# hynkis/Python-MPC

Measured on AMD Instinct MI355X. Metric: QP solves/sec (batch) at N=20 nx=4 nu=1, higher is better.
Workload: dtype f64

## Files before the change

### python-mpc_amd/csrc/device_common.h

```cpp
#pragma once
#include <hip/hip_runtime.h>

#include "kernels.h"

#ifdef MPCQP_SKEW
__device__ inline __attribute__((convergent)) void mpcqp_skew_barrier() {
    __builtin_amdgcn_fence(__ATOMIC_RELEASE, "workgroup");
    __builtin_amdgcn_s_barrier();
    __builtin_amdgcn_fence(__ATOMIC_ACQUIRE, "workgroup");
    const unsigned w = __builtin_amdgcn_readfirstlane(threadIdx.x >> 6);
    const unsigned t = (unsigned)(__builtin_amdgcn_s_memtime() >> 3);
    if (((t ^ (w * 0x9E3779B9u)) >> 7) & 1u) __builtin_amdgcn_s_sleep(20);
}
#define __syncthreads() mpcqp_skew_barrier()
#endif

namespace mpcqp {

#define OSQP_INFTY 1e30
#define MIN_SCALING 1e-4
#define MAX_SCALING 1e4
#define RHO_MIN 1e-6
#define RHO_MAX 1e6
#define RHO_TOL 1e-4
// ... 26 lines not shown
template <int CTRL>
__device__ __forceinline__ double dpp(double v) {
    int lo = __double2loint(v), hi = __double2hiint(v);
    lo = __builtin_amdgcn_mov_dpp(lo, CTRL, 0xF, 0xF, true);
    hi = __builtin_amdgcn_mov_dpp(hi, CTRL, 0xF, 0xF, true);
    return __hiloint2double(hi, lo);
}

__device__ __forceinline__ double reduce8(double v) {
    v += dpp<0xB1>(v);
    v += dpp<0x4E>(v);
    v += dpp<0x141>(v);
    return v;
}

__device__ __forceinline__ double reduce16(double v) {
    v += dpp<0xB1>(v);
    v += dpp<0x4E>(v);
    v += dpp<0x141>(v);
    v += dpp<0x140>(v);
    return v;
}

template <int CTRL, int RM>
__device__ __forceinline__ double dpp_rows(double v) {
    int lo = __double2loint(v), hi = __double2hiint(v);
    lo = __builtin_amdgcn_mov_dpp(lo, CTRL, RM, 0xF, true);
    hi = __builtin_amdgcn_mov_dpp(hi, CTRL, RM, 0xF, true);
    return __hiloint2double(hi, lo);
}

__device__ __forceinline__ double reduce32_hi(double v) {
    v = reduce16(v);
    v += dpp_rows<0x142, 0xA>(v);
    return v;
}

__device__ __forceinline__ double lane63(double v) {
    return __hiloint2double(__builtin_amdgcn_readlane(__double2hiint(v), 63),
                            __builtin_amdgcn_readlane(__double2loint(v), 63));
}
__device__ __forceinline__ double wave_max(double v) {
    v = cmax(v, dpp<0xB1>(v));
    v = cmax(v, dpp<0x4E>(v));
    v = cmax(v, dpp<0x141>(v));
    v = cmax(v, dpp<0x140>(v));
    v = cmax(v, dpp_rows<0x142, 0xA>(v));
    v = cmax(v, dpp_rows<0x143, 0xC>(v));
    return lane63(v);
}
__device__ __forceinline__ double wave_sum(double v) {
    v = reduce16(v);
    v += dpp_rows<0x142, 0xA>(v);
    v += dpp_rows<0x143, 0xC>(v);
    return lane63(v);
}

template <int TT, int K>
__device__ __forceinline__ void block_max(double (&v)[K], double* red) {
    if constexpr (TT == 64) {
#pragma unroll
        for (int k = 0; k < K; ++k) v[k] = wave_max(v[k]);
    } else {
        constexpr int NW = TT / 64;
        const int wid = threadIdx.x >> 6, lane = threadIdx.x & 63;
#pragma unroll
        for (int k = 0; k < K; ++k) {
            const double r = wave_max(v[k]);
            if (lane == 0) red[wid * K + k] = r;
        }
        __syncthreads();
#pragma unroll
        for (int k = 0; k < K; ++k) {
            double r = red[k];
#pragma unroll
            for (int w = 1; w < NW; ++w) r = cmax(r, red[w * K + k]);
            v[k] = r;
        }
        __syncthreads();
    }
}

template <int TT, int K>
__device__ __forceinline__ void block_max_to(const double (&v)[K], double* red, double* out) {
    constexpr int NW = TT / 64;
    const int wid = threadIdx.x >> 6, lane = threadIdx.x & 63, t = threadIdx.x;
#pragma unroll
    for (int k = 0; k < K; ++k) {
        const double r = wave_max(v[k]);
        if (lane == 0) red[wid * K + k] = r;
    }
    __syncthreads();
    if (t < K) {
        double r = red[t];
#pragma unroll
        for (int w = 1; w < NW; ++w) r = cmax(r, red[w * K + t]);
        out[t] = r;
    }
    __syncthreads();
}

template <int TT, int K>
__device__ __forceinline__ void block_sum(double (&v)[K], double* red) {
    if constexpr (TT == 64) {
#pragma unroll
        for (int k = 0; k < K; ++k) v[k] = wave_sum(v[k]);
    } else {
        constexpr int NW = TT / 64;
        const int wid = threadIdx.x >> 6, lane = threadIdx.x & 63;
#pragma unroll
        for (int k = 0; k < K; ++k) {
            const double r = wave_sum(v[k]);
            if (lane == 0) red[wid * K + k] = r;
        }
        __syncthreads();
#pragma unroll
        for (int k = 0; k < K; ++k) {
            double r = red[k];
            if constexpr (NW == 4) {
                r = (red[k] + red[K + k]) + (red[2 * K + k] + red[3 * K + k]);
            } else {
#pragma unroll
                for (int w = 1; w < NW; ++w) r += red[w * K + k];
            }
            v[k] = r;
        }
        __syncthreads();
    }
}

__device__ __forceinline__ double vmax(double a, double b) { return __builtin_fmax(a, b); }

template <int CTRL, int K>
__device__ __forceinline__ void tmax_step(const double (&in)[K], double (&out)[(K + 1) / 2], bool upper) {
    constexpr int H = (K + 1) / 2;
#pragma unroll
    for (int j = 0; j < H; ++j) {
        const double lo = in[j];
        const double hi = j + H < K ? in[j + H] : 0.0;
        out[j] = vmax(upper ? hi : lo, dpp<CTRL>(upper ? lo : hi));
    }
}

template <bool HALF>
__device__ __forceinline__ double xmax_swap(double v) {
    const unsigned lo = (unsigned)__double2loint(v), hi = (unsigned)__double2hiint(v);
    const auto l = HALF ? __builtin_amdgcn_permlane32_swap(lo, lo, false, false)
                        : __builtin_amdgcn_permlane16_swap(lo, lo, false, false);
    const auto h = HALF ? __builtin_amdgcn_permlane32_swap(hi, hi, false, false)
                        : __builtin_amdgcn_permlane16_swap(hi, hi, false, false);
    return vmax(__hiloint2double((int)h[0], (int)l[0]), __hiloint2double((int)h[1], (int)l[1]));
}

template <int TT, int K, int KS>
__device__ __forceinline__ void block_max_sum_tr(double (&v)[K], double (&sm)[KS], double* red) {
    constexpr int NW = TT / 64, K1 = (K + 1) / 2, K2 = (K1 + 1) / 2;
    const int lane = threadIdx.x & 63, wid = threadIdx.x >> 6;
    double t1[K1], t2[K2];
    tmax_step<0xB1, K>(v, t1, lane & 1);
    tmax_step<0x4E, K1>(t1, t2, (lane >> 1) & 1);
#pragma unroll
    for (int j = 0; j < K2; ++j) {
        double x = t2[j];
        x = vmax(x, dpp<0x124>(x));
        x = vmax(x, dpp<0x128>(x));
        x = xmax_swap<false>(x);
        x = xmax_swap<true>(x);
        t2[j] = x;
    }
    double s[KS];
#pragma unroll
    for (int k = 0; k < KS; ++k) s[k] = wave_sum(sm[k]);
    double* rs = red + 4 * NW * K2;
    if (lane < 4) {
        int lq = lane;
        asm volatile("" : "+v"(lq));
#pragma unroll
        for (int j = 0; j < K2; ++j) red[(lq * K2 + j) * NW + wid] = t2[j];
    }
    if (lane == 0) {
        int wq = wid;
        asm volatile("" : "+v"(wq));
#pragma unroll
        for (int k = 0; k < KS; ++k) rs[wq * KS + k] = s[k];
    }
    __syncthreads();
    if constexpr (NW > 4) {
        double* const fin = rs + NW * KS;
        if ((int)threadIdx.x < K) {
            const int k = threadIdx.x, b0 = k >= K1, r1 = k - K1 * b0, b1 = r1 >= K2, j = r1 - K2 * b1;
            const double* src = red + ((b0 + 2 * b1) * K2 + j) * NW;
            double r = src[0];
#pragma unroll
            for (int w = 1; w < NW; ++w) r = vmax(r, src[w]);
            fin[k] = r;
        }
        __syncthreads();
#pragma unroll
        for (int k = 0; k < K; ++k) v[k] = fin[k];
    } else {
#pragma unroll
        for (int k = 0; k < K; ++k) {
            const int b0 = k >= K1, r1 = k - K1 * b0, b1 = r1 >= K2, j = r1 - K2 * b1;
            const double* src = red + ((b0 + 2 * b1) * K2 + j) * NW;
            double r = src[0];
#pragma unroll
            for (int w = 1; w < NW; ++w) r = vmax(r, src[w]);
            v[k] = r;
        }
    }
#pragma unroll
    for (int k = 0; k < KS; ++k) {
        double r = rs[k];
        if constexpr (NW == 4) {
            r = (rs[k] + rs[KS + k]) + (rs[2 * KS + k] + rs[3 * KS + k]);
        } else {
#pragma unroll
            for (int w = 1; w < NW; ++w) r += rs[w * KS + k];
        }
        sm[k] = r;
    }
    __syncthreads();
}

template <int TT>
__device__ __forceinline__ void order_epilogue(const KParams& p, int* smem) {
    const long B = gridDim.x;
    if (!p.done || !p.order || B <= p.slots || B > kOrderFuseMax) return;
    const int tid = threadIdx.x;
    int* cnt = smem;
    int* last = smem + 256;
    __syncthreads();
    if (tid == 0) {
        __threadfence();
        *last = atomicAdd(p.done, 1) == (int)(B - 1);
        __threadfence();
    }
    __syncthreads();
    if (!*last) return;
    int shift = 0;
    while ((p.max_iter >> shift) >= 256) ++shift;
    const int* iter = p.iter;
    int* order = const_cast<int*>(p.order);
    auto bin = [&](long i) {
        const int k = __builtin_nontemporal_load(iter + i) >> shift;
        return 255 - (k < 255 ? k : 255);
    };
    for (int k = tid; k < 256; k += TT) cnt[k] = 0;
    __syncthreads();
    for (long i = tid; i < B; i += TT) atomicAdd(&cnt[bin(i)], 1);
    __syncthreads();
    if (tid == 0) {
        int s = 0;
        for (int k = 0; k < 256; ++k) {
            const int c = cnt[k];
            cnt[k] = s;
            s += c;
        }
        *p.done = 0;
    }
    __syncthreads();
    for (long i = tid; i < B; i += TT) order[atomicAdd(&cnt[bin(i)], 1)] = (int)i;
}

template <int TT>
__device__ __forceinline__ bool block_any(bool f, int* flag) {
    if constexpr (TT == 64) {
        return __builtin_amdgcn_ballot_w64(f) != 0;
    } else {
        if (threadIdx.x == 0) *flag = 0;
        __syncthreads();
        if (f) *flag = 1;
        __syncthreads();
        bool r = *flag != 0;
        __syncthreads();
        return r;
    }
}

}
```

### python-mpc_amd/csrc/solve_wave.hip

```cpp
#include <hip/hip_runtime.h>

#include <algorithm>
#include <cstdlib>
#include <type_traits>

#include "setup_r.h"
#include "solve_phases.h"
#include "wave_util.h"

namespace mpcqp {

[[maybe_unused]] constexpr int TW = 64;

#ifdef MPCQP_EXPERIMENTAL
struct WaveFactor {
    double SB[2][S];
    __device__ __forceinline__ void load(const double* __restrict__ Sg) {
        const int lane = threadIdx.x, h = lane >> 5, r = lane & 31;
#pragma unroll
        for (int e = 0; e < 2; ++e) {
            const double* src = Sg + (long)(e ? 3 - h : h) * SS + r * S;
#pragma unroll
            for (int c = 0; c < S; ++c) SB[e][c] = src[c];
        }
// ... 855 lines not shown
#endif
            p.prof[b * kProfSlots + 6] = clock64() - t0c;
            p.prof[b * kProfSlots + 7] = wall_clock64() - t0w;
            p.prof[b * kProfSlots + 15] = t0w;
        }
    }
#endif
#undef PH
#undef PHL
#undef PHC
}

template <int K, int RS, int KPK, int K1>
__global__ __launch_bounds__(T2, 1) void k_solve_w2(KParams p, double* __restrict__ xo, double* __restrict__ yo,
                                                    int factor_only) {
    solve_w2_body<K, RS, KPK, K1>(p, xo, yo, factor_only);
    extern __shared__ __attribute__((aligned(16))) double sm[];
    order_epilogue<T2>(p, (int*)sm);
}

template <int K, int RS, int KPK, int K1, int SK, int SRS, int SAS, int SPS>
__global__ __launch_bounds__(T2, 1) void k_setup_solve_w2(KParams p, const double* __restrict__ Px_in,
                                                          const double* __restrict__ Ax_in,
                                                          const double* __restrict__ q_in,
                                                          const double* __restrict__ l_in,
                                                          const double* __restrict__ u_in, double* __restrict__ xo,
                                                          double* __restrict__ yo) {
    extern __shared__ __attribute__((aligned(16))) double sm[];
    setup_r_body<T2, SK, 4, SRS, SAS, SPS>(p, instance_of(p), Px_in, Ax_in, q_in, l_in, u_in, sm);
    __syncthreads();
    solve_w2_body<K, RS, KPK, K1>(p, xo, yo, 0);
    order_epilogue<T2>(p, (int*)sm);
}

constexpr int T4 = 256;

template <int QR, int NB0, int NB1>
__device__ __forceinline__ void form_dense_rows(__attribute__((address_space(1))) dpair* kd, const double* Sg,
                                                const double* gl, int a, int lane) {
    constexpr int NP = 6, T4_ = 256, TC = 8;
    auto pidx = [](int x, int y) { return y < x ? x * (x - 1) / 2 + y : NP; };
    const int bq = lane >> 4, l16 = lane & 15, i0 = 4 * (l16 >> 1);
    const double* const Ta = Sg + a * SS;
    const int nbs = (bq >> 1) ? NB1 : NB0, jb = (bq >> 1) ? NB0 : 0;
    const unsigned t0 = (unsigned)(a * 64 + (bq & 1) * 32 + i0);
#pragma unroll 1
    for (int pass = 0; pass < 2; ++pass) {
        const int c0 = 16 * (l16 & 1) + TC * pass;
        double acc[4][TC];
        {
            const double* src = Sg + bq * SS + i0 * S + c0;
            const bool diag = bq == a;
#pragma unroll
            for (int i = 0; i < 4; ++i)
#pragma unroll
                for (int c = 0; c < TC; c += 2) {
                    double v0, v1;
                    ld2(src + i * S + c, v0, v1);
                    acc[i][c] = diag ? v0 : 0.0;
                    acc[i][c + 1] = diag ? v1 : 0.0;
                }
        }
        auto step = [&](const double (&cf)[4], const double* row) __attribute__((always_inline)) {
            double rv[TC];
#pragma unroll
            for (int c = 0; c < TC; c += 2) ld2(row + c, rv[c], rv[c + 1]);
#pragma unroll
            for (int i = 0; i < 4; ++i)
#pragma unroll
                for (int c = 0; c < TC; ++c) acc[i][c] += cf[i] * rv[c];
        };
        if (a > 0) {
            const double* g = gl + pidx(a, bq) * 8 * S + c0;
#pragma unroll
            for (int q = 0; q < QR; ++q) {
                double cf[4];
#pragma unroll
                for (int i = 0; i < 4; ++i) cf[i] = Ta[(i0 + i) * S + q];
                step(cf, g + q * S);
            }
        }
        if (a < 3) {
            const double* g = gl + pidx(bq, a) * 8 * S + i0;
            const double* Tb = Sg + bq * SS + c0;
#pragma unroll
            for (int q = 0; q < QR; ++q) {
                double cf[4];
                ld2(g + q * S, cf[0], cf[1]);
                ld2(g + q * S + 2, cf[2], cf[3]);
                step(cf, Tb + q * S);
            }
        }
#pragma unroll 1
        for (int k = a + 1; k < 4; ++k) {
            const double* gka = gl + pidx(k, a) * 8 * S + i0;
            const double* gkb = gl + pidx(k, bq) * 8 * S + c0;
            const double* Tk = Sg + k * SS;
            double V[4][QR];
#pragma unroll
            for (int i = 0; i < 4; ++i)
#pragma unroll
                for (int q = 0; q < QR; ++q) V[i][q] = 0.0;
#pragma unroll
            for (int pp = 0; pp < QR; ++pp) {
                double g[4];
                ld2(gka + pp * S, g[0], g[1]);
                ld2(gka + pp * S + 2, g[2], g[3]);
#pragma unroll
                for (int q = 0; q < QR; ++q) {
                    const double t = Tk[pp * S + q];
#pragma unroll
                    for (int i = 0; i < 4; ++i) V[i][q] += g[i] * t;
                }
            }
#pragma unroll
            for (int q = 0; q < QR; ++q) {
                const double cf[4] = {V[0][q], V[1][q], V[2][q], V[3][q]};
                step(cf, gkb + q * S);
            }
        }
#pragma unroll
        for (int c = 0; c < TC; c += 2) {
            if (c0 + c < nbs) {
                const unsigned jp = (unsigned)((jb + c0 + c) >> 1);
#pragma unroll
                for (int i = 0; i < 4; ++i) {
                    kd[jp * T4_ + t0 + i].x = acc[i][c];
                    kd[jp * T4_ + t0 + i].y = acc[i][c + 1];
                }
            }
        }
    }
}

template <int K, int KPK, int QR, bool EL = false, int KC = K, bool DK = false, bool RU = false, bool ONE = false,
          int GL = 0>
__device__ __forceinline__ void solve_w4_body(const KParams& p, double* __restrict__ xo, double* __restrict__ yo,
                                              int factor_only = 0) {
    static_assert(!(DK && EL), "the dense inverse covers plans without eliminated columns");
    const int tid = threadIdx.x, w = __builtin_amdgcn_readfirstlane(tid >> 6), lane = tid & 63;
    const int h = lane >> 5, r = lane & 31;
    constexpr int NB = 4, NP = NB * (NB - 1) / 2;
    static_assert(KC % 2 == 0, "the rhs splits the column list over the half-waves");
    constexpr int KH = KC / 2;
    constexpr int LE = 2;
    const long b = instance_of(p);
    const int n = p.n, m = p.m, npad = p.npad, nnzP = p.nnzP, nnzA = p.nnzA;
    SL2 C = carve(p);
    SLds& L = C.L;
    const double* Hg = GL == 1 ? C.L.Acsc + 2 * ((lds_base_bytes(p) + 15) / 16) + (long)NB * SS
                           : p.H + b * (long)p.nb * SS;
    double* const Sg = C.L.Acsc + 2 * ((lds_base_bytes(p) + 15) / 16);
    constexpr bool SWZ = ONE && GL == 1 && !EL && !DK && QR <= 5;

    if (p.err[b]) {
        for (int j = tid; j < n; j += T4) if (xo) xo[b * n + j] = __builtin_nan("");
        for (int i = tid; i < m; i += T4) if (yo) yo[b * m + i] = __builtin_nan("");
        if (tid == 0) fail_status(p, b);
        return;
    }
#ifdef MPCQP_PHASE_PROF
    long long tph = 0, t0c = 0, t0w = 0;
    const bool prof = p.prof != nullptr;
    if (prof) { t0w = wall_clock64(); t0c = tph = clock64(); if (tid < 16) L.pacc[tid] = 0; }
#define PH(k) if (prof && tid == 0) { const long long t_ = clock64(); L.pacc[k] += t_ - tph; tph = t_; }
#else
#define PH(k)
#endif
    constexpr bool OPQ = EL || QR > 5;
    auto cscal = [&](int k) __attribute__((always_inline)) {
        return OPQ ? opaque_gptr(p.scal + b * 4)[k] : p.scal[b * 4 + k];
    };
    double rho = p.scal[b * 4 + 2];
    const double sigma = p.sigma, alpha = p.alpha;
    const bool warm = !ONE && p.warm_start != 0;
    const int mp = solve_mpad(m);
    if constexpr (!ONE) {
        for (int e = tid; e < nnzA; e += T4) L.Acsc[e] = p.Ax[b * nnzA + e];
        if (tid == 0) L.Acsc[nnzA] = 0.0;
        for (int v = tid; v < nnzP; v += T4) L.Pv[v] = p.Px[b * nnzP + v];
        if (tid == 0) L.Pv[nnzP] = 0.0;
        for (int i = tid; i < mp; i += T4) {
            const bool in = i < m;
            L.lo[i] = in ? p.l[b * m + i] : 0.0;
            L.up[i] = in ? p.u[b * m + i] : 0.0;
            L.ct[i] = in ? p.ct[b * m + i] : 0;
            C.Z[i] = (in && warm) ? p.z[b * m + i] : 0.0;
        }
        for (int pc = tid; pc < npad; pc += T4) {
            L.qv[pc] = p.q[b * npad + pc];
            C.X[pc] = warm ? p.x[b * npad + pc] : 0.0;
        }
    } else {
        if (tid == 0) L.Acsc[nnzA] = 0.0;
        if (tid == 0) L.Pv[nnzP] = 0.0;
        if constexpr (GL == 2)
            for (int o = tid; o < (NP + 1) * 8 * S; o += T4) L.gl[o] = 0.0;
    }
    if (tid < 8) L.cor[tid] = 0.0;
    if (tid < 8) L.cor[32 + tid] = 0.0;
    if (tid < 16) L.res[tid] = 0.0;
    if (tid < 4) L.flag[tid] = 0;

    int status = MPCQP_UNSOLVED_, rho_updates = 0, iter = 0, info_iter = 0;
    bool can_check = false, need_factor = true;
    const bool low = h == 0;
    const int pe0 = (EL && !low) ? p.eown[w * S + r] : -1;
    const bool colv = low && p.pad_var[w * S + r] >= 0;
    double* const Fo = p.F + b * (long)p.nb * SS;
    double ec = 0.0, ed = 0.0;
    const unsigned abase = lds_addr(L.Acsc), wbase = lds_addr(L.w), xbase = lds_addr(L.xt);
    const unsigned Xbase = lds_addr(C.X);
    GatherW<K> rg;
    GatherW<KH> chs;
    GatherW<LE> el;
    const bool rows_wave = w * 64 < mp;
    constexpr int NB0 = 26, NB1 = 28;
    static_assert(!DK || (NB0 + NB1) * T4 == kDenseRowDoubles, "KParams::Kd rows");
    double Kr[DK ? NB0 + NB1 : 1];
    constexpr int DKW = 8;
    PH(5)
    for (;;) {
        const int tid = OPQ ? opaque_v(threadIdx.x) : (int)threadIdx.x;
        const int lane = tid & 63, h = lane >> 5, r = lane & 31, rr = lane >> 3, ch = lane & 7;
        const int pc = w * S + r;
        const int pe = OPQ ? opaque_v(pe0) : pe0;
        const int xc = pe >= 0 ? pe : pc;
        const int ri = min(tid, mp - 1);
        __syncthreads();
        if (need_factor) {
            need_factor = false;
            if (iter > 0) {
                if constexpr (GL == 1) {
                    double* const ysv = Sg + (long)NB * SS + (long)(NB * (NB - 1) / 2) * p.amax * S;
                    for (int i = tid; i < m; i += T4) ysv[i] = L.ys[i];
                } else {
                    const auto yp = opaque_gptr(p.y + b * m);
                    for (int i = tid; i < m; i += T4) yp[i] = L.ys[i];
                }
                __syncthreads();
            }
            bool ok;
            if constexpr (RU) {
                if (iter == 0 && p.reuse && p.ffresh[b] == 1 && p.scal[b * 4 + 3] == rho) {
                    const double2* src = (const double2*)(p.Si + b * (long)p.nb * SS);
                    for (int e = tid; e < 2 * SS; e += T4) ((double2*)Sg)[e] = src[e];
                    ok = true;
                } else if constexpr (EL) {
                    ok = factorize_lds_nl<T4, EL>(p.self, b, rho);
                } else {
                    ok = factorize_nl<T4, EL>(p.self, b, rho, Sg);
                }
                __syncthreads();
                if (tid == 0) p.ffresh[b] = 0;
            } else if constexpr (GL == 1) {
                ok = factorize_g_nl<T4, EL, SWZ>(p.self, b, rho);
            } else if constexpr (GL == 2) {
                ok = factorize_gl_nl<T4, EL>(p.self, b, rho);
            } else if constexpr (EL) {
                ok = factorize_lds_nl<T4, EL>(p.self, b, rho);
            } else {
                ok = factorize_nl<T4, EL>(p.self, b, rho, Sg);
            }
            if (!ok) {
                if (iter == 0) {
                    if (xo) for (int j = tid; j < n; j += T4) opaque_ptr(xo + b * n)[j] = __builtin_nan("");
                    if (yo) for (int i = tid; i < m; i += T4) opaque_ptr(yo + b * m)[i] = __builtin_nan("");
                    if (tid == 0) fail_status(p, b);
                    return;
                }
                status = MPCQP_NON_CVX_;
                can_check = true;
                break;
            }
            if (factor_only) {
                __syncthreads();
                double2* dst = (double2*)(p.Si + b * (long)p.nb * SS);
                for (int e = tid; e < 2 * SS; e += T4) dst[e] = ((const double2*)Sg)[e];
                if (tid == 0) {
                    p.ffresh[b] = 1;
                    p.scal[b * 4 + 3] = rho;
                }
                return;
            }
            __syncthreads();
            const bool have_y = iter > 0 || warm;
            if constexpr (GL == 1) {
                const double* const ysv = Sg + (long)NB * SS + (long)(NB * (NB - 1) / 2) * p.amax * S;
                for (int i = tid; i < mp; i += T4) L.ys[i] = (have_y && i < m) ? ysv[i] : 0.0;
            } else {
                const auto yp = opaque_gptr(p.y + b * m);
                for (int i = tid; i < mp; i += T4) L.ys[i] = (have_y && i < m) ? yp[i] : 0.0;
            }
            if constexpr (GL != 2) {
                for (int o = tid; o < (NP + 1) * 8 * S; o += T4) {
                    const int q = o >> 8, t = (o >> 5) & 7;
                    L.gl[o] = (q < NP && t < p.amax) ? Hg[(long)q * p.amax * S + (o & 255)] : 0.0;
                }
            }
            chs.load(p.gcol + (h ? KH : 0) * npad + pc, npad, abase, wbase);
            if constexpr (EL) {
                if (pe >= 0) {
                    el.load(p.gcol + pe, npad, abase, wbase);
                    const int e = pe - p.nb * S;
                    ec = Fo[2 * e];
                    ed = Fo[2 * e + 1];
                } else {
                    el.clear(abase + 8u * nnzA, wbase);
                }
            }
            if (ri < m) rg.load(p.grow + ri, m, abase, xbase);
            else rg.clear(abase + 8u * nnzA, xbase);
            if constexpr (DK) {
                __syncthreads();
                form_dense_rows<QR, NB0, NB1>((__attribute__((address_space(1))) dpair*)opaque_gptr(
                                                  p.Kd + b * kDenseRowDoubles),
                                              Sg, L.gl, w, lane);
                __syncthreads();
            }
            PH(0)
        }
        if constexpr (DK) {
            const auto kd = (const __attribute__((address_space(1))) dpair*)opaque_gptr(p.Kd + b * kDenseRowDoubles);
#pragma unroll
            for (int j = 0; j < NB0 + NB1; j += 2) {
                Kr[j] = kd[(unsigned)((j / 2) * T4 + tid)].x;
                Kr[j + 1] = kd[(unsigned)((j / 2) * T4 + tid)].y;
            }
        }
        double SB[16];
        if constexpr (SWZ) {
            const double* src = Sg + (long)w * SS;
            const int rs = opaque_v(r);
#pragma unroll
            for (int c = 0; c < 16; c += 2) ld2(src + tile_at<true>(rs, 16 * h + c), SB[c], SB[c + 1]);
        } else if constexpr (!DK) {
            const double* src = Sg + (long)w * SS + r * S + 16 * h;
#pragma unroll
            for (int c = 0; c < 16; c += 2) ld2(src + c, SB[c], SB[c + 1]);
        }
        double X = C.X[xc], DX = 0.0;
        const double Q = L.qv[xc];
        int gslot[2], tslot[2];
        {
            int pr[2] = {NP, NP}, jj[2] = {3, 3};
            if (w == 0) {
                if (h == 0) { pr[0] = 0; jj[0] = 1; pr[1] = 1; jj[1] = 2; }
                else        { pr[0] = 3; jj[0] = 3; }
            } else if (w == 1) {
                if (h == 0) { pr[0] = 2; jj[0] = 2; }
                else        { pr[0] = 4; jj[0] = 3; }
            } else if (w == 2) {
                if (h == 0) { pr[0] = 5; jj[0] = 3; }
            }
#pragma unroll
            for (int s = 0; s < 2; ++s) {
                gslot[s] = lds_addr(L.gl + pr[s] * 8 * S + r);
                tslot[s] = lds_addr(L.tv + jj[s] * 8);
            }
        }
        const int nsw = (NB - w) >> 1;
        const GatherW<KH>& ch2 = chs;
        double ca[KH];
#pragma unroll
        for (int k = 0; k < KH; ++k) ca[k] = lds_at(ch2.e[k] & 0xFFFFu);
        double ea[LE];
#pragma unroll
        for (int k = 0; k < LE; ++k) ea[k] = EL ? lds_at(el.e[k] & 0xFFFFu) : 0.0;
        double bj = 0.0;
        const double r_hi = RHO_EQ_OVER_RHO_INEQ * rho;
        double y = L.ys[ri], Z = C.Z[ri], dy = 0.0;
        double av[K];
#pragma unroll
        for (int k = 0; k < K; ++k) av[k] = DK ? 0.0 : lds_at(rg.e[k] & 0xFFFFu);
        const double rlo = L.lo[ri], rup = L.up[ri];
        const signed char cl = L.ct[ri];
        const double rv = cl < 0 ? RHO_MIN : (cl > 0 ? r_hi : rho);
        const double rvi = cl < 0 ? 1.0 / RHO_MIN : (cl > 0 ? 1.0 / r_hi : 1.0 / rho);
        __syncthreads();
        double ga[NB - 1][4];
        if constexpr (!DK) {
            const double* gq = L.gl + (w * (w - 1) / 2) * 8 * S + rr * S + 4 * ch;
#pragma unroll
            for (int j = 0; j < NB - 1; ++j) {
                if (j < w) {
                    ld2(gq + j * 8 * S, ga[j][0], ga[j][1]);
                    ld2(gq + j * 8 * S + 2, ga[j][2], ga[j][3]);
                } else {
                    ga[j][0] = ga[j][1] = ga[j][2] = ga[j][3] = 0.0;
                }
            }
        }
        double gc[2][QR];
        if constexpr (!DK) {
#pragma unroll
            for (int s = 0; s < 2; ++s)
#pragma unroll
                for (int q = 0; q < QR; ++q) gc[s][q] = s < nsw ? lds_at(gslot[s] + q * S * 8) : 0.0;
        }
        if (rows_wave) L.w[ri] = rv * Z - y;
        int stop_at = p.max_iter;
        if (p.check_term) stop_at = min(stop_at, (iter / p.check_term + 1) * p.check_term);
        if (p.adaptive_rho && p.rho_interval) stop_at = min(stop_at, (iter / p.rho_interval + 1) * p.rho_interval);
        __syncthreads();
        PH(5)
        double* const cw = L.cor + w * 8;
        const double* const cwh = L.cor + (h ? 32 : w * 8);
        while (iter < stop_at) {
            ++iter;
            {
                double wv[KH];
#pragma unroll
                for (int k = 0; k < KH; ++k) wv[k] = lds_at(ch2.e[k] >> 16);
                double v;
                if constexpr (EL) {
                    double we[LE];
#pragma unroll
                    for (int k = 0; k < LE; ++k) we[k] = lds_at(el.e[k] >> 16);
                    bj = sigma * X - Q;
#pragma unroll
                    for (int k = 0; k < LE; ++k) bj += ea[k] * we[k];
                    v = low ? bj : -(ec * bj);
                } else {
                    v = low ? sigma * X - Q : 0.0;
                }
#pragma unroll
                for (int k = 0; k < KH; ++k) v += ca[k] * wv[k];
                const unsigned vlo = (unsigned)__double2loint(v), vhi = (unsigned)__double2hiint(v);
                const auto l2 = __builtin_amdgcn_permlane32_swap(vlo, vlo, false, false);
                const auto h2 = __builtin_amdgcn_permlane32_swap(vhi, vhi, false, false);
                const double v0 = __hiloint2double((int)h2[0], (int)l2[0]);
                const double v1 = __hiloint2double((int)h2[1], (int)l2[1]);
                if (low) L.rb[pc] = colv ? v0 + v1 : 0.0;
            }
            __syncthreads();
            PH(1)
            if constexpr (DK) {
                const double* const rbh = L.rb + S * h;
                double a[4] = {0.0, 0.0, 0.0, 0.0};
                constexpr int NE = NB0 + NB1, NWIN = (NE + DKW - 1) / DKW;
                double v[2][DKW];
                auto issue = [&](int k, double (&dst)[DKW]) __attribute__((always_inline)) {
#pragma unroll
                    for (int c = 0; c < DKW; c += 2) {
                        const int e = k * DKW + c;
                        if (e < NE) ld2(rbh + (e < NB0 ? e : 2 * S + e - NB0), dst[c], dst[c + 1]);
                    }
                };
                issue(0, v[0]);
#pragma unroll
                for (int k = 0; k < NWIN; ++k) {
                    if (k + 1 < NWIN) issue(k + 1, v[(k + 1) & 1]);
                    __builtin_amdgcn_sched_barrier(0);
#pragma unroll
                    for (int c = 0; c < DKW; ++c)
                        if (k * DKW + c < NE) a[c & 3] += Kr[k * DKW + c] * v[k & 1][c];
                    __builtin_amdgcn_sched_barrier(0);
                }
                const double th = (a[0] + a[1]) + (a[2] + a[3]);
                const unsigned lo = (unsigned)__double2loint(th), hi = (unsigned)__double2hiint(th);
                const auto l2 = __builtin_amdgcn_permlane32_swap(lo, lo, false, false);
                const auto h2 = __builtin_amdgcn_permlane32_swap(hi, hi, false, false);
                const double xn = __hiloint2double((int)h2[0], (int)l2[0]) + __hiloint2double((int)h2[1], (int)l2[1]);
                if (low) L.xt[pc] = xn;
                const double xnew = alpha * xn + (1.0 - alpha) * X;
                DX = xnew - X;
                X = xnew;
            } else {
            if (w > 0) {
                double acc[NB - 1] = {0.0, 0.0, 0.0};
#pragma unroll
                for (int j = 0; j < NB - 1; ++j) {
                    if (j < w) {
                        double bj[4];
                        ld2(L.rb + j * S + 4 * ch, bj[0], bj[1]);
                        ld2(L.rb + j * S + 4 * ch + 2, bj[2], bj[3]);
#pragma unroll
                        for (int e = 0; e < 4; ++e) acc[j] += ga[j][e] * bj[e];
                    }
                }
                cw[rr] = reduce8((acc[0] + acc[1]) + acc[2]);
            }
            __builtin_amdgcn_fence(__ATOMIC_RELEASE, "wavefront");
            __builtin_amdgcn_wave_barrier();
            __builtin_amdgcn_fence(__ATOMIC_ACQUIRE, "wavefront");
            PH(12)
            double t;
            {
                constexpr int QE = (QR + 1) & ~1;
                double v[16], cc[QE];
#pragma unroll
                for (int c = 0; c < 16; c += 2) ld2(L.rb + w * S + 16 * h + c, v[c], v[c + 1]);
#pragma unroll
                for (int c = 0; c < QE; c += 2) ld2(cwh + c, cc[c], cc[c + 1]);
#pragma unroll
                for (int c = 0; c < QR; ++c) v[c] += cc[c];
                double a[4] = {0.0, 0.0, 0.0, 0.0};
#pragma unroll
                for (int c = 0; c < 16; ++c) a[c & 3] += SB[c] * v[c];
                const double th = (a[0] + a[1]) + (a[2] + a[3]);
                const unsigned lo = (unsigned)__double2loint(th), hi = (unsigned)__double2hiint(th);
                const auto l2 = __builtin_amdgcn_permlane32_swap(lo, lo, false, false);
                const auto h2 = __builtin_amdgcn_permlane32_swap(hi, hi, false, false);
                const double t0 = __hiloint2double((int)h2[0], (int)l2[0]);
                const double t1 = __hiloint2double((int)h2[1], (int)l2[1]);
                t = t0 + t1;
                if (low && r < 8) L.tv[w * 8 + r] = t;
            }
            __syncthreads();
            PH(13)
            {
                constexpr int QE = (QR + 1) & ~1;
                double gv[2][QE], tq[2][QE];
#pragma unroll
                for (int s = 0; s < 2; ++s) {
                    if (s < nsw) {
#pragma unroll
                        for (int q = 0; q < QE; ++q) gv[s][q] = q < QR ? gc[s][q] : 0.0;
#pragma unroll
                        for (int q = 0; q < QE; q += 2) lds_at2(tslot[s] + q * 8, tq[s][q], tq[s][q + 1]);
                    } else {
#pragma unroll
                        for (int q = 0; q < QE; ++q) gv[s][q] = tq[s][q] = 0.0;
                    }
                }
                double a0 = 0.0, a1 = 0.0;
#pragma unroll
                for (int s = 0; s < 2; ++s)
#pragma unroll
                    for (int q = 0; q < QR; q += 2) {
                        a0 += gv[s][q] * tq[s][q];
                        if (q + 1 < QR) a1 += gv[s][q + 1] * tq[s][q + 1];
                    }
                const double d = a0 + a1;
                const unsigned lo = (unsigned)__double2loint(d), hi = (unsigned)__double2hiint(d);
                const auto l2 = __builtin_amdgcn_permlane32_swap(lo, lo, false, false);
                const auto h2 = __builtin_amdgcn_permlane32_swap(hi, hi, false, false);
                const double d0 = __hiloint2double((int)h2[0], (int)l2[0]);
                const double d1 = __hiloint2double((int)h2[1], (int)l2[1]);
                const double xn = t + (d0 + d1);
                if (low) L.xt[pc] = xn;
                double xl = xn;
                if constexpr (EL) {
                    if (!low) {
                        xl = ed * bj - ec * xn;
                        if (pe >= 0) L.xt[pe] = xl;
                    }
                }
                const double xnew = alpha * xl + (1.0 - alpha) * X;
                DX = xnew - X;
                X = xnew;
            }
            }
            __syncthreads();
            PH(14)
            if (rows_wave) {
                double xv[K], ar[K];
#pragma unroll
                for (int k = 0; k < K; ++k) xv[k] = lds_at(rg.e[k] >> 16);
#pragma unroll
                for (int k = 0; k < K; ++k) ar[k] = DK ? lds_at(rg.e[k] & 0xFFFFu) : av[k];
                const double lo = rlo, up = rup;
                double zt = ar[0] * xv[0];
#pragma unroll
                for (int k = 1; k < K; ++k) zt += ar[k] * xv[k];
                const double zr = alpha * zt + (1.0 - alpha) * Z;
                const double zn = __builtin_fmin(__builtin_fmax(zr + rvi * y, lo), up);
                const double dd = rv * (zr - zn);
                Z = zn;
                dy = dd;
                y += dd;
                L.w[ri] = rv * zn - y;
            }
            __syncthreads();
            PH(3)
        }
        if (low) { lds_put(C.X, pc, X); lds_put(L.dx, pc, DX); }
        if (EL && pe >= 0) { lds_put(C.X, pe, X); lds_put(L.dx, pe, DX); }
        if (rows_wave) { lds_put(L.ys, ri, y); lds_put(C.Z, ri, Z); lds_put(C.dY, ri, dy); }
        __syncthreads();
        can_check = p.check_term && (iter % p.check_term == 0);
        const bool do_rho = p.adaptive_rho && p.rho_interval && (iter % p.rho_interval == 0);
        if (!can_check && !do_rho) break;
        info_iter = iter;
        bool stop = false;
        {
            const int col = EL ? (low ? pc : pe) : pc;
            const bool cv = col >= 0 && (EL || low) && opaque_gptr(p.pad_var)[col] >= 0;
            GatherW<KC> cg;
            GatherW<KPK> pg;
            if (col >= 0) {
                cg.load(p.gcol + col, npad, abase, wbase);
                pg.load(p.gpsym + col, npad, lds_addr(L.Pv), Xbase);
            } else {
                cg.clear(abase + 8u * nnzA, wbase);
                pg.clear(lds_addr(L.Pv) + 8u * nnzP, Xbase);
            }
            const int oz = opaque_zero();
            double Dv, Ev;
            if constexpr (GL == 1) {
                Dv = col >= 0 ? edl_D(p, C)[col] : 1.0;
                Ev = ri < m ? edl_E(p, C)[ri] : 1.0;
            } else {
                Dv = col >= 0 ? opaque_gptr(p.D + b * npad)[col] : 1.0;
                Ev = ri < m ? opaque_gptr(p.E + b * m)[ri] : 1.0;
            }
            const bool unscale = p.scaling && !p.scaled_term;
            const unsigned ysbase = lds_addr(L.ys), dYbase = lds_addr(C.dY), dxbase = lds_addr(L.dx);
            double mx[17], sm[2] = {0.0, 0.0}, adx = 0.0;
#pragma unroll
            for (int k = 0; k < 17; ++k) mx[k] = 0.0;
            {
                const bool ok = tid < m;
                double ax = 0.0, ad = 0.0;
#pragma unroll
                for (int k = 0; k < K; ++k) {
                    const unsigned e = rg.e[k], va = e >> 16;
                    const double a = lds_at(e & 0xFFFFu);
                    ax += a * lds_at(va - xbase + Xbase);
                    ad += a * lds_at(va - xbase + dxbase);
                }
                adx = ad;
                const double zi = Z, pr = ax - zi, ei = 1.0 / Ev;
                const double lo = L.lo[ri], up = L.up[ri];
                double d = dy;
                if (up > OSQP_INFTY * MIN_SCALING) d = (lo < -OSQP_INFTY * MIN_SCALING) ? 0.0 : cmin(d, 0.0);
                else if (lo < -OSQP_INFTY * MIN_SCALING) d = cmax(d, 0.0);
                if (ok) {
                    mx[0] = fabs(ei * pr);
                    mx[2] = fabs(ei * zi);
                    mx[3] = fabs(ei * ax);
                    mx[7] = fabs(pr);
                    mx[9] = fabs(zi);
                    mx[10] = fabs(ax);
                    mx[14] = fabs(unscale ? Ev * d : d);
                    sm[0] = up * cmax(d, 0.0) + lo * cmin(d, 0.0);
                    C.dY[ri] = d;
                }
            }
            {
                double px = 0.0, pdx = 0.0, aty = 0.0;
#pragma unroll
                for (int k = 0; k < KPK; ++k) {
                    const unsigned e = pg.e[k], va = e >> 16;
                    const double pv = lds_at(e & 0xFFFFu);
                    px += pv * lds_at(va);
                    pdx += pv * lds_at(va - Xbase + dxbase);
                }
#pragma unroll
                for (int k = 0; k < KC; ++k) {
                    const unsigned e = cg.e[k];
                    aty += lds_at(e & 0xFFFFu) * lds_at((e >> 16) - wbase + ysbase);
                }
                if (cv) {
                    const double d = (Q + px) + aty, di = 1.0 / Dv;
                    mx[1] = fabs(di * d);
                    mx[4] = fabs(di * Q);
                    mx[5] = fabs(di * aty);
                    mx[6] = fabs(di * px);
                    mx[8] = fabs(d);
                    mx[11] = fabs(Q);
                    mx[12] = fabs(aty);
                    mx[13] = fabs(px);
                    mx[15] = fabs(unscale ? Dv * DX : DX);
                    mx[16] = fabs(unscale ? pdx * di : pdx);
                }
            }
            if (tid < npad && opaque_gptr(p.pad_var)[tid] >= 0) sm[1] = L.qv[tid + oz] * L.dx[tid + oz];
            if (do_rho || !unscale) {
                block_max_sum_tr<T4, 17, 2>(mx, sm, L.red);
            } else {
                double m10[10] = {mx[0], mx[1], mx[2], mx[3], mx[4], mx[5], mx[6], mx[14], mx[15], mx[16]};
                block_max_sum_tr<T4, 10, 2>(m10, sm, L.red);
#pragma unroll
                for (int k = 0; k < 7; ++k) mx[k] = m10[k];
                mx[14] = m10[7];
                mx[15] = m10[8];
                mx[16] = m10[9];
            }
            Res R;
            if (unscale) {
                R.pri = mx[0]; R.dua = cscal(1) * mx[1];
                R.nz = mx[2]; R.nax = mx[3]; R.nq = mx[4]; R.naty = mx[5]; R.npx = mx[6];
            } else {
                R.pri = mx[7]; R.dua = mx[8];
                R.nz = mx[9]; R.nax = mx[10]; R.nq = mx[11]; R.naty = mx[12]; R.npx = mx[13];
            }
            R.rpri = mx[7]; R.rdua = mx[8]; R.rz = mx[9]; R.rax = mx[10]; R.rq = mx[11]; R.raty = mx[12]; R.rpx = mx[13];
            if (m == 0) R.pri = 0.0;
            if (tid == 0) R.save(L.res);
            if (can_check) {
                int st = MPCQP_UNSOLVED_;
                bool done = false;
                if (R.pri > OSQP_INFTY || R.dua > OSQP_INFTY) {
                    st = MPCQP_NON_CVX_;
                    done = true;
                } else {
                    const bool prim_ok = m == 0 || R.pri < p.eps_abs + p.eps_rel * cmax(R.nz, R.nax);
                    double mxd = cmax(cmax(R.nq, R.naty), R.npx);
                    if (unscale) mxd *= cscal(1);
                    const bool dual_ok = R.dua < p.eps_abs + p.eps_rel * mxd;
                    bool prim_inf = false, dual_inf = false;
                    if (!prim_ok || !dual_ok) {
                        const double norm_dy = mx[14], norm_dx = mx[15], epi = p.eps_pinf, edi = p.eps_dinf;
                        const double cs = unscale ? cscal(0) : 1.0;
                        if (!prim_ok && m != 0 && norm_dy > epi && sm[0] < epi * norm_dy) {
                            __syncthreads();
                            double na[1] = {0.0};
                            double a = 0.0;
#pragma unroll
                            for (int k = 0; k < KC; ++k) {
                                const unsigned e = cg.e[k];
                                a += lds_at(e & 0xFFFFu) * lds_at((e >> 16) - wbase + dYbase);
                            }
                            if (cv) na[0] = fabs(unscale ? a * (1.0 / Dv) : a);
                            block_max<T4, 1>(na, L.red);
                            prim_inf = na[0] < epi * norm_dy;
                        }
                        if (!dual_ok && norm_dx > edi && sm[1] < cs * edi * norm_dx && mx[16] < cs * edi * norm_dx) {
                            bool viol = false;
                            if (tid < m) {
                                const double ar = unscale ? adx * (1.0 / Ev) : adx;
                                const double lo = L.lo[ri], up = L.up[ri];
                                if ((up < OSQP_INFTY * MIN_SCALING && ar > edi * norm_dx) ||
                                    (lo > -OSQP_INFTY * MIN_SCALING && ar < -edi * norm_dx))
                                    viol = true;
                            }
                            dual_inf = !block_any<T4>(viol, L.flag);
                        }
                    }
                    if (prim_ok && dual_ok) {
                        st = MPCQP_SOLVED_;
                        done = true;
                    } else if (prim_inf) {
                        st = MPCQP_PRIMAL_INFEASIBLE_;
                        if (tid == 0) L.flag[3] = unscale;
                        done = true;
                    } else if (dual_inf) {
                        st = MPCQP_DUAL_INFEASIBLE_;
                        if (tid == 0) L.flag[2] = unscale;
                        done = true;
                    }
                }
                __syncthreads();
                if (done && tid == 0) L.flag[1] = st;
                __syncthreads();
                status = done ? st : MPCQP_UNSOLVED_;
                stop = done;
            }
        }
        if (!stop && do_rho) {
            Res R;
            R.restore(L.res);
            const double pr = R.rpri / (cmax(R.rz, R.rax) + DIVISION_TOL);
            const double du = R.rdua / (cmax(cmax(R.rq, R.raty), R.rpx) + DIVISION_TOL);
            double rn = rho * sqrt(pr / (du + DIVISION_TOL));
            rn = cmin(cmax(rn, RHO_MIN), RHO_MAX);
            if (rn > rho * p.rho_tol || rn < rho / p.rho_tol) {
                rho = cmin(cmax(rn, RHO_MIN), RHO_MAX);
                rho_updates++;
                need_factor = true;
            }
        }
        __syncthreads();
        PH(4)
        if (stop || iter >= p.max_iter) break;
    }
    const double cval = cscal(0), cinv = cscal(1);
    if (!can_check && status == MPCQP_UNSOLVED_) {
        update_info_nl<T4, GL == 1>(p.self, b, cinv);
        info_iter = iter;
        status = check_termination_nl<T4, GL == 1>(p.self, b, cval, cinv, 0);
    }
    const bool has_sol = !(status == MPCQP_PRIMAL_INFEASIBLE_ || status == MPCQP_PRIMAL_INFEASIBLE_INACCURATE_ ||
                           status == MPCQP_DUAL_INFEASIBLE_ || status == MPCQP_DUAL_INFEASIBLE_INACCURATE_ ||
                           status == MPCQP_NON_CVX_);
    if (has_sol) objective_nl<T4>(p.self, cinv);
    if (status == MPCQP_UNSOLVED_) {
        status = check_termination_nl<T4, GL == 1>(p.self, b, cval, cinv, 1);
        if (status == MPCQP_UNSOLVED_) status = MPCQP_MAX_ITER_REACHED_;
    }
    finalize_nl<T4, ONE, GL == 1>(p.self, b, xo, yo, cinv, rho, status, info_iter, rho_updates, p.ostat, p.oiter);
#ifdef MPCQP_PHASE_PROF
    if (prof) {
        __syncthreads();
        PH(5)
        if (tid == 0) {
#pragma unroll
            for (int k = 0; k < 6; ++k) p.prof[b * kProfSlots + k] = L.pacc[k];
#pragma unroll
            for (int k = 8; k < 15; ++k) p.prof[b * kProfSlots + k] = L.pacc[k];
            p.prof[b * kProfSlots + 2] = L.pacc[12] + L.pacc[13] + L.pacc[14];
            p.prof[b * kProfSlots + 6] = clock64() - t0c;
            p.prof[b * kProfSlots + 7] = wall_clock64() - t0w;
            p.prof[b * kProfSlots + 15] = t0w;
        }
    }
#endif
#undef PH
}

template <int K, int KPK, int QR, bool EL = false, int KC = K, bool FO = false, bool DK = false>
__global__ __launch_bounds__(T4, 2) void k_solve_w4(KParams p, double* __restrict__ xo, double* __restrict__ yo,
                                                    int ) {
    solve_w4_body<K, KPK, QR, EL, KC, DK, !FO && !DK>(p, xo, yo, FO ? 1 : 0);
    extern __shared__ __attribute__((aligned(16))) double sm[];
    order_epilogue<T4>(p, (int*)sm);
}

template <int K, int KPK, int QR, int SK, int SAS, bool EL = false, int KC = K, bool DK = false, bool ONE = false,
          int GL = 0>
__global__ __launch_bounds__(T4, 2) void k_setup_solve_w4(KParams p, const double* __restrict__ Px_in,
                                                          const double* __restrict__ Ax_in,
                                                          const double* __restrict__ q_in,
                                                          const double* __restrict__ l_in,
                                                          const double* __restrict__ u_in, double* __restrict__ xo,
                                                          double* __restrict__ yo) {
    extern __shared__ __attribute__((aligned(16))) double sm[];
    setup_r_body<T4, SK, 4, 1, SAS, 1, false, ONE, GL == 1>(p, instance_of(p), Px_in, Ax_in, q_in, l_in, u_in, sm);
    __syncthreads();
    solve_w4_body<K, KPK, QR, EL, KC, DK, false, ONE, GL>(p, xo, yo);
    order_epilogue<T4>(p, (int*)sm);
}


#ifdef MPCQP_EXPERIMENTAL
constexpr int T8 = 512;

template <int K, int KPK>
__device__ __forceinline__ void solve_w8_body(const KParams& p, double* __restrict__ xo, double* __restrict__ yo,
                                              int factor_only) {
    const int tid = threadIdx.x, w = __builtin_amdgcn_readfirstlane(tid >> 6), lane = tid & 63;
    const int h = lane >> 5, r = lane & 31, rr = lane >> 2, ch = lane & 3;
    constexpr int NB = 8, NP = NB * (NB - 1) / 2;
    constexpr int QR = 12, GR = 12;
    static_assert(K % 2 == 0, "the rhs splits the column list over the half-waves");
    constexpr int KH = K / 2;
    const long b = instance_of(p);
    const int n = p.n, m = p.m, npad = p.npad, nnzP = p.nnzP, nnzA = p.nnzA;
    SL2 C = carve(p);
    SLds& L = C.L;
    double* const Hg = p.H + b * (long)p.nb * SS;
    double* const Fg = p.F + b * (long)p.nb * SS;
    double* const Sg = L.SP + w8_toff(p.amax);
    double* const red8 = L.SP + w8_roff(p.m, p.npad, p.amax);

    if (p.err[b]) {
        for (int j = tid; j < n; j += T8) if (xo) xo[b * n + j] = __builtin_nan("");
        for (int i = tid; i < m; i += T8) if (yo) yo[b * m + i] = __builtin_nan("");
        if (tid == 0) fail_status(p, b);
        return;
    }
#ifdef MPCQP_PHASE_PROF
    long long tph = 0, t0c = 0, t0w = 0;
    const bool prof = p.prof != nullptr;
    if (prof) { t0w = wall_clock64(); t0c = tph = clock64(); if (tid < 16) L.pacc[tid] = 0; }
#define PH(k) if (prof && tid == 0) { const long long t_ = clock64(); L.pacc[k] += t_ - tph; tph = t_; }
#else
#define PH(k)
#endif
    const double cval = p.scal[b * 4 + 0], cinv = p.scal[b * 4 + 1];
    double rho = p.scal[b * 4 + 2];
    const double sigma = p.sigma, alpha = p.alpha;
    const bool warm = p.warm_start != 0;
    for (int e = tid; e < nnzA; e += T8) L.Acsc[e] = p.Ax[b * nnzA + e];
    if (tid == 0) L.Acsc[nnzA] = 0.0;
    for (int v = tid; v < nnzP; v += T8) L.Pv[v] = p.Px[b * nnzP + v];
    if (tid == 0) L.Pv[nnzP] = 0.0;
    const int mp = solve_mpad(m);
    for (int i = tid; i < mp; i += T8) {
        const bool in = i < m;
        L.lo[i] = in ? p.l[b * m + i] : 0.0;
        L.up[i] = in ? p.u[b * m + i] : 0.0;
        L.ct[i] = in ? p.ct[b * m + i] : 0;
        C.Z[i] = (in && warm) ? p.z[b * m + i] : 0.0;
    }
    for (int pc = tid; pc < npad; pc += T8) {
        L.qv[pc] = p.q[b * npad + pc];
        C.X[pc] = warm ? p.x[b * npad + pc] : 0.0;
    }
    if (tid < 16) L.cor[tid] = 0.0;
    if (tid < 16) L.cor[128 + tid] = 0.0;
    if (tid < 16) L.res[tid] = 0.0;
    if (tid < 4) L.flag[tid] = 0;

    int status = MPCQP_UNSOLVED_, rho_updates = 0, iter = 0, info_iter = 0;
    bool can_check = false, need_factor = true;
    const int pc = w * S + r;
    const bool low = h == 0;
    const unsigned abase = lds_addr(L.Acsc), wbase = lds_addr(L.w), xbase = lds_addr(L.xt);
    const unsigned Xbase = lds_addr(C.X);
    bool cv = false;
    double Dv = 1.0, Ev = 1.0;
    GatherW<K> cg, rg;
    GatherW<KPK> pg;
    const int ri = min(tid, mp - 1);
    const bool rows_wave = w * 64 < mp;
    double SB[16];
#pragma unroll
    for (int c = 0; c < 16; ++c) SB[c] = 0.0;
    PH(5)
    for (;;) {
        __syncthreads();
        if (need_factor) {
            need_factor = false;
            if (iter > 0) {
                for (int i = tid; i < m; i += T8) p.y[b * m + i] = L.ys[i];
                __syncthreads();
            }
            const bool ok = factorize_nl<T8>(p.self, b, rho, Sg);
            if (!ok) {
                if (iter == 0) {
                    for (int j = tid; j < n; j += T8) if (xo) xo[b * n + j] = __builtin_nan("");
                    for (int i = tid; i < m; i += T8) if (yo) yo[b * m + i] = __builtin_nan("");
                    if (tid == 0) fail_status(p, b);
                    return;
                }
                status = MPCQP_NON_CVX_;
                can_check = true;
                break;
            }
            if (factor_only) return;
            __syncthreads();
            {
                const double* src = Sg + (long)w * SS + r * S + 16 * h;
#pragma unroll
                for (int c = 0; c < 16; c += 2) ld2(src + c, SB[c], SB[c + 1]);
            }
            __syncthreads();
            const bool have_y = iter > 0 || warm;
            for (int i = tid; i < mp; i += T8) L.ys[i] = (have_y && i < m) ? p.y[b * m + i] : 0.0;
            for (int o = tid; o < (NP + 1) * GR * S; o += T8) {
                const int q = o / (GR * S), t = (o >> 5) - q * GR;
                L.gl[o] = (q < NP && t < p.amax) ? w8_gpair(Fg, Hg, p.amax, q)[t * S + (o & 31)] : 0.0;
            }
            cv = low && p.pad_var[pc] >= 0;
            cg.load(p.gcol + pc, npad, abase, wbase);
            pg.load(p.gpsym + pc, npad, lds_addr(L.Pv), Xbase);
            Dv = p.D[b * npad + pc];
            Ev = ri < m ? p.E[b * m + ri] : 1.0;
            if (ri < m) rg.load(p.grow + ri, m, abase, xbase);
            else rg.clear(abase + 8u * nnzA, xbase);
            PH(0)
        }
        double X = C.X[pc], DX = 0.0;
// ... 534 lines not shown
```

Measured before the change: 2.569 million.

## Lean termination path: lane-broadcast reduction, direct LDS factor reads, fewer barriers

For the swizzled single-instance plan, the block max/sum reduction now has each lane finish one result and broadcasts all results via readlane, removing the final shared-memory pass. The per-refactor copy of the factor tiles into L.gl is skipped; gather coefficients are read directly from the factor stored in LDS. The column gather reuses already-loaded half-wave data through a permlane32 swap instead of reloading it. Residuals are kept in registers for the rho update, and two barriers around the status flag are removed. Phase-profiling slots are extended. The risk is correctness of the removed barriers and the lane-indexed reduction.

```diff
diff --git a/python-mpc_amd/csrc/device_common.h b/python-mpc_amd/csrc/device_common.h
--- a/python-mpc_amd/csrc/device_common.h
+++ b/python-mpc_amd/csrc/device_common.h
@@ -202,9 +202,10 @@
     return vmax(__hiloint2double((int)h[0], (int)l[0]), __hiloint2double((int)h[1], (int)l[1]));
 }
 
-template <int TT, int K, int KS>
+template <int TT, int K, int KS, bool LANE = false>
 __device__ __forceinline__ void block_max_sum_tr(double (&v)[K], double (&sm)[KS], double* red) {
     constexpr int NW = TT / 64, K1 = (K + 1) / 2, K2 = (K1 + 1) / 2;
+    static_assert(!LANE || (NW == 4 && K + KS <= 64), "the lane form: four waves, a lane per result");
     const int lane = threadIdx.x & 63, wid = threadIdx.x >> 6;
     double t1[K1], t2[K2];
     tmax_step<0xB1, K>(v, t1, lane & 1);
@@ -235,6 +236,31 @@
         for (int k = 0; k < KS; ++k) rs[wq * KS + k] = s[k];
     }
     __syncthreads();
+    if constexpr (LANE) {
+        int lq = lane;
+        asm volatile("" : "+v"(lq));
+        const int k = lq < K ? lq : 0, b0 = k >= K1, r1 = k - K1 * b0, b1 = r1 >= K2, j = r1 - K2 * b1;
+        const double* src = red + ((b0 + 2 * b1) * K2 + j) * NW;
+        double r = src[0];
+#pragma unroll
+        for (int w = 1; w < NW; ++w) r = vmax(r, src[w]);
+        const int ks = (lq >= K && lq < K + KS) ? lq - K : 0;
+        const double s4 = (rs[ks] + rs[KS + ks]) + (rs[2 * KS + ks] + rs[3 * KS + ks]);
+        const double res = lq < K ? r : s4;
+        const int lo = __double2loint(res), hi = __double2hiint(res);
+#pragma unroll
+        for (int q = 0; q < K; ++q) {
+            v[q] = __hiloint2double(__builtin_amdgcn_readlane(hi, q), __builtin_amdgcn_readlane(lo, q));
+            asm volatile("" : "+v"(v[q]));
+        }
+#pragma unroll
+        for (int q = 0; q < KS; ++q) {
+            sm[q] = __hiloint2double(__builtin_amdgcn_readlane(hi, K + q), __builtin_amdgcn_readlane(lo, K + q));
+            asm volatile("" : "+v"(sm[q]));
+        }
+        __syncthreads();
+        return;
+    }
     if constexpr (NW > 4) {
         double* const fin = rs + NW * KS;
         if ((int)threadIdx.x < K) {
diff --git a/python-mpc_amd/csrc/solve_wave.hip b/python-mpc_amd/csrc/solve_wave.hip
--- a/python-mpc_amd/csrc/solve_wave.hip
+++ b/python-mpc_amd/csrc/solve_wave.hip
@@ -1031,6 +1031,7 @@
                            : p.H + b * (long)p.nb * SS;
     double* const Sg = C.L.Acsc + 2 * ((lds_base_bytes(p) + 15) / 16);
     constexpr bool SWZ = ONE && GL == 1 && !EL && !DK && QR <= 5;
+    constexpr bool LEAN = SWZ;
 
     if (p.err[b]) {
         for (int j = tid; j < n; j += T4) if (xo) xo[b * n + j] = __builtin_nan("");
@@ -1171,7 +1172,7 @@
                 const auto yp = opaque_gptr(p.y + b * m);
                 for (int i = tid; i < mp; i += T4) L.ys[i] = (have_y && i < m) ? yp[i] : 0.0;
             }
-            if constexpr (GL != 2) {
+            if constexpr (GL != 2 && !LEAN) {
                 for (int o = tid; o < (NP + 1) * 8 * S; o += T4) {
                     const int q = o >> 8, t = (o >> 5) & 7;
                     L.gl[o] = (q < NP && t < p.amax) ? Hg[(long)q * p.amax * S + (o & 255)] : 0.0;
@@ -1221,6 +1222,7 @@
         double X = C.X[xc], DX = 0.0;
         const double Q = L.qv[xc];
         int gslot[2], tslot[2];
+        bool gz[2];
         {
             int pr[2] = {NP, NP}, jj[2] = {3, 3};
             if (w == 0) {
@@ -1234,7 +1236,9 @@
             }
 #pragma unroll
             for (int s = 0; s < 2; ++s) {
-                gslot[s] = lds_addr(L.gl + pr[s] * 8 * S + r);
+                gslot[s] = LEAN ? lds_addr(Hg + (pr[s] < NP ? pr[s] : 0) * p.amax * S + r)
+                                : lds_addr(L.gl + pr[s] * 8 * S + r);
+                gz[s] = pr[s] == NP;
                 tslot[s] = lds_addr(L.tv + jj[s] * 8);
             }
         }
@@ -1255,10 +1259,21 @@
         const double rlo = L.lo[ri], rup = L.up[ri];
         const signed char cl = L.ct[ri];
         const double rv = cl < 0 ? RHO_MIN : (cl > 0 ? r_hi : rho);
-        const double rvi = cl < 0 ? 1.0 / RHO_MIN : (cl > 0 ? 1.0 / r_hi : 1.0 / rho);
+        const double rvi = LEAN ? 1.0 / rv : (cl < 0 ? 1.0 / RHO_MIN : (cl > 0 ? 1.0 / r_hi : 1.0 / rho));
         __syncthreads();
         double ga[NB - 1][4];
-        if constexpr (!DK) {
+        if constexpr (LEAN) {
+            const int gs = p.amax * S * 8;
+            const unsigned gq = lds_addr(Hg) + (w * (w - 1) / 2) * gs + (rr * S + 4 * ch) * 8;
+#pragma unroll
+            for (int j = 0; j < NB - 1; ++j) {
+                ga[j][0] = ga[j][1] = ga[j][2] = ga[j][3] = 0.0;
+                if (j < w && rr < p.amax) {
+                    lds_at2(gq + j * gs, ga[j][0], ga[j][1]);
+                    lds_at2(gq + j * gs + 16, ga[j][2], ga[j][3]);
+                }
+            }
+        } else if constexpr (!DK) {
             const double* gq = L.gl + (w * (w - 1) / 2) * 8 * S + rr * S + 4 * ch;
 #pragma unroll
             for (int j = 0; j < NB - 1; ++j) {
@@ -1271,7 +1286,13 @@
             }
         }
         double gc[2][QR];
-        if constexpr (!DK) {
+        if constexpr (LEAN) {
+#pragma unroll
+            for (int s = 0; s < 2; ++s)
+#pragma unroll
+                for (int q = 0; q < QR; ++q)
+                    gc[s][q] = (s < nsw && !gz[s] && q < p.amax) ? lds_at(gslot[s] + q * S * 8) : 0.0;
+        } else if constexpr (!DK) {
 #pragma unroll
             for (int s = 0; s < 2; ++s)
 #pragma unroll
@@ -1282,7 +1303,7 @@
         if (p.check_term) stop_at = min(stop_at, (iter / p.check_term + 1) * p.check_term);
         if (p.adaptive_rho && p.rho_interval) stop_at = min(stop_at, (iter / p.rho_interval + 1) * p.rho_interval);
         __syncthreads();
-        PH(5)
+        PH(15)
         double* const cw = L.cor + w * 8;
         const double* const cwh = L.cor + (h ? 32 : w * 8);
         while (iter < stop_at) {
@@ -1463,12 +1484,21 @@
         if (!can_check && !do_rho) break;
         info_iter = iter;
         bool stop = false;
+        Res Rk;
         {
             const int col = EL ? (low ? pc : pe) : pc;
-            const bool cv = col >= 0 && (EL || low) && opaque_gptr(p.pad_var)[col] >= 0;
+            const bool cv = LEAN ? colv : col >= 0 && (EL || low) && opaque_gptr(p.pad_var)[col] >= 0;
             GatherW<KC> cg;
             GatherW<KPK> pg;
-            if (col >= 0) {
+            if constexpr (LEAN) {
+#pragma unroll
+                for (int k = 0; k < KH; ++k) {
+                    const auto e2 = __builtin_amdgcn_permlane32_swap(chs.e[k], chs.e[k], false, false);
+                    cg.e[k] = e2[0];
+                    cg.e[KH + k] = e2[1];
+                }
+                pg.load(p.gpsym + col, npad, lds_addr(L.Pv), Xbase);
+            } else if (col >= 0) {
                 cg.load(p.gcol + col, npad, abase, wbase);
                 pg.load(p.gpsym + col, npad, lds_addr(L.Pv), Xbase);
             } else {
@@ -1546,17 +1576,19 @@
                 }
             }
             if (tid < npad && opaque_gptr(p.pad_var)[tid] >= 0) sm[1] = L.qv[tid + oz] * L.dx[tid + oz];
+            PH(6)
             if (do_rho || !unscale) {
-                block_max_sum_tr<T4, 17, 2>(mx, sm, L.red);
+                block_max_sum_tr<T4, 17, 2, LEAN>(mx, sm, L.red);
             } else {
                 double m10[10] = {mx[0], mx[1], mx[2], mx[3], mx[4], mx[5], mx[6], mx[14], mx[15], mx[16]};
-                block_max_sum_tr<T4, 10, 2>(m10, sm, L.red);
+                block_max_sum_tr<T4, 10, 2, LEAN>(m10, sm, L.red);
 #pragma unroll
                 for (int k = 0; k < 7; ++k) mx[k] = m10[k];
                 mx[14] = m10[7];
                 mx[15] = m10[8];
                 mx[16] = m10[9];
             }
+            PH(7)
             Res R;
             if (unscale) {
                 R.pri = mx[0]; R.dua = cscal(1) * mx[1];
@@ -1568,6 +1600,7 @@
             R.rpri = mx[7]; R.rdua = mx[8]; R.rz = mx[9]; R.rax = mx[10]; R.rq = mx[11]; R.raty = mx[12]; R.rpx = mx[13];
             if (m == 0) R.pri = 0.0;
             if (tid == 0) R.save(L.res);
+            if constexpr (LEAN) Rk = R;
             if (can_check) {
                 int st = MPCQP_UNSOLVED_;
                 bool done = false;
@@ -1621,16 +1654,17 @@
                         done = true;
                     }
                 }
-                __syncthreads();
+                if constexpr (!LEAN) __syncthreads();
                 if (done && tid == 0) L.flag[1] = st;
-                __syncthreads();
+                if constexpr (!LEAN) __syncthreads();
                 status = done ? st : MPCQP_UNSOLVED_;
                 stop = done;
             }
         }
         if (!stop && do_rho) {
             Res R;
-            R.restore(L.res);
+            if constexpr (LEAN) R = Rk;
+            else R.restore(L.res);
             const double pr = R.rpri / (cmax(R.rz, R.rax) + DIVISION_TOL);
             const double du = R.rdua / (cmax(cmax(R.rq, R.raty), R.rpx) + DIVISION_TOL);
             double rn = rho * sqrt(pr / (du + DIVISION_TOL));
@@ -1670,6 +1704,11 @@
 #pragma unroll
             for (int k = 8; k < 15; ++k) p.prof[b * kProfSlots + k] = L.pacc[k];
             p.prof[b * kProfSlots + 2] = L.pacc[12] + L.pacc[13] + L.pacc[14];
+            p.prof[b * kProfSlots + 4] = L.pacc[4] + L.pacc[6] + L.pacc[7];
+            p.prof[b * kProfSlots + 5] = L.pacc[5] + L.pacc[15];
+            p.prof[b * kProfSlots + 16] = L.pacc[6];
+            p.prof[b * kProfSlots + 17] = L.pacc[7];
+            p.prof[b * kProfSlots + 18] = L.pacc[15];
             p.prof[b * kProfSlots + 6] = clock64() - t0c;
             p.prof[b * kProfSlots + 7] = wall_clock64() - t0w;
             p.prof[b * kProfSlots + 15] = t0w;
```

Result: faster. 2.622 million (median of 6 runs) (+2.1%).
